# jkbonfield/htscodecs

Hardware: AMD Instinct MI355X
Metric: MB/s uncompressed throughput (encode+decode), rANS4x16 order-1, q40 blocks (higher is better)
Workload: dtype u8/u32; 1 GPU; rANS4x16 order-1 encode+decode, 23040 x 1048576 B q40+dir blocks per GPU (cyclic tiles of tests/dat/q40+dir), device-resident; order=1, blocks_per_gpu=23040, block_size=1048576

## Files before the change

### htscodecs_amd/csrc/r4x16_enc_chain.h

```cpp
#pragma once
#include <stdlib.h>
#include <type_traits>
#include "r4x16_dev.h"
#include "r4x16_sched.h"
#include "r4x16_enc_step.h"

template <int ORDER>
__device__ __forceinline__ u32 chain_encode(gcu8 *data, u32 n, gcu8 *image, u32 ns, u32 bits, gcu32 *rcptab,
                                            gu8 *scratch_end, bool active, u32 lane)
{
    const u32 k = lane & 3;
    GAS const u16 *cum = (GAS const u16 *)(image + ENC_IMG_IDX);
    const u32 rs = ns + 1;
    u32 x = RANS_LOW;
    u32 written = 0;
    u32 nsteps, first;
    u32 p;
    const u32 q = n >> 2;
    if (ORDER == 0) {
        const u32 gtop = n ? (n - 1) >> 2 : 0;
        nsteps = n ? gtop + 1 : 0;
        first = (4 * gtop + k < n) ? 0 : 1;
        p = 4 * (gtop - (first ? 1 : 0)) + k;
    } else {
        const u32 tail = n - 4 * q;
        nsteps = tail + q;
        first = (k == 3) ? 0 : tail;
        p = (k == 3) ? n - 1 : k * q + q - 1;
    }
    if (!active) { nsteps = 0; first = 0; }

    u32 cur = 0;
    if (nsteps > first) cur = image[data[p]];

    for (u32 s = 0; wave_any(s < nsteps); s++) {
        const bool live = s >= first && s < nsteps;
        bool emit = false;
        u32 rcp = 0, pk = 0, nextc = 0;
        if (live) {
            u32 row = 0;
            if (ORDER == 0) {
                if (p >= 4) nextc = image[data[p - 4]];
            } else if (s != nsteps - 1) {
                nextc = image[data[p - 1]];
                row = nextc;
            }
            const u32 c0 = cum[row * rs + cur], c1 = cum[row * rs + cur + 1];
            pk = c0 | ((c1 - c0) << 16);
            rcp = enc_rcp(rcptab, c1 - c0);
            emit = enc_wants_emit(x, pk, bits);
        }
        const u32 em = quad_ballot(emit, lane);
        if (emit) {
            const u32 above = __popc(em >> (k + 1));
            *(gu16 *)(scratch_end - 2 * (written + above + 1)) = (u16)x;
            x >>= 16;
        }
        written += __popc(em);
        if (live) {
            x = enc_advance(x, rcp, pk, bits);
            cur = nextc;
            p -= (ORDER == 0) ? 4 : 1;
        }
    }
    if (active) *(gu32 *)(scratch_end - 2 * written - 16 + 4 * k) = x;
    return active ? 2 * written + 16 : 0;
}

#define ENC_LRCP_BYTES 16400u
#define ENC_LFREQ_BYTES   8208u
static_assert(ENC_LFREQ_BYTES >= 8u * ENC_FREQTAB_ENTRIES && ENC_LFREQ_BYTES % 16u == 0, "frequency table in LDS");
template <bool BYTE>
struct EncOutT {
    u8 *ring;
    u32 ring126;
    gu8 *send;
    gu8 *dump;
    u32 written;
    u32 flushed;
    u32 k, lane;
    bool active;
    u32x4 held;
    gu8 *held_dst;
    u32 above = (0xeu << k) & 0xfu;
    static constexpr u32 HALF_SHIFT = BYTE ? 6u : 5u;
    __device__ __forceinline__ u32 emit16(u32 x, bool live, bool over)
    {
        const u64 m = __ballot(over) & __ballot(live);
        const u32 em = (u32)(m >> (lane & ~3u)) & 0xfu;
        const bool emit = live && over;
        const u32 j = written + __popc(em >> (k + 1));
        const u32 j63 = emit ? (j & 63u) : ~0u;
        *(LAS u16 *)(unsigned long)(ring126 - 2u * j63) = (u16)x;
        written += __popc(em);
        return emit ? x >> 16 : x;
    }
    template <bool ALL>
    __device__ __forceinline__ u32 emit16q(u32 x, bool live, bool over)
    {
        const u64 m = ALL ? __ballot(over) : __ballot(over) & __ballot(live);
        const u32 em = (u32)(m >> (lane & ~3u));
        const bool emit = ALL ? over : live && over;
        const u32 j = written + __popc(em & above);
        const u32 j63 = emit ? (j & 63u) : ~0u;
        u32 a;
        asm("v_mad_i32_i24 %0, %1, -2, %2" : "=v"(a) : "v"(j63), "v"(ring126));
        *(LAS u16 *)(unsigned long)a = (u16)x;
        written += __popc(em & 0xfu);
        return emit ? x >> 16 : x;
    }
    template <bool Q = false, bool ALL = false>
    __device__ __forceinline__ void step(u32 &x, bool live, u32 rcp, u32 pk, u32 bits)
    {
        const u32 f = pk >> 16, start = pk & 0xffffu;
        u32 xs;
        if (BYTE) {
            const u32 x_max = f << 19;
            const bool o1 = x >= x_max, o2 = (x >> 8) >= x_max;
            const u64 lv = __ballot(live);
            const u32 e1 = (u32)((__ballot(o1) & lv) >> (lane & ~3u)) & 0xfu, e2 = (u32)((__ballot(o2) & lv) >> (lane & ~3u)) & 0xfu;
            const bool emit1 = live && o1, emit2 = live && o2;
            const u32 j = written + __popc(e1 >> (k + 1)) + __popc(e2 >> (k + 1));
            const u32 j1 = emit1 ? (j & 127u) : ~0u, j2 = emit2 ? ((j + 1u) & 127u) : ~0u;
            *(LAS u8 *)(unsigned long)(ring126 - j1) = (u8)x;
            *(LAS u8 *)(unsigned long)(ring126 - j2) = (u8)(x >> 8);
            xs = emit2 ? x >> 16 : emit1 ? x >> 8 : x;
            written += __popc(e1) + __popc(e2);
        } else xs = Q ? emit16q<ALL>(x, live, x >= (f << (31u - bits))) : emit16(x, live, x >= (f << (31u - bits)));
        const u32 fm1 = f - 1u;
        const u32 rsh = 31u - (u32)__clz((int)(fm1 | 1u));
        const u32 q = (__umulhi(xs, rcp) >> rsh) + (fm1 == 0u ? 1u : 0u);
        const u32 cmpl = (1u << bits) - f;
        const u32 xn = __umul24(q, cmpl) + (xs + start);
        x = ALL || live ? xn : xs;
    }
    template <bool ALL = false>
    __device__ __forceinline__ void step_freq(u32 &x, bool live, u32 m, u32 w, u32 start, u32 f)
    {
        const u32 xs = emit16q<ALL>(x, live, x >= (f << 21));
        const u32 q = (__umulhi(xs, m) + xs) >> ((w >> 24) & 31u);
        const u32 xn = __umul24(q, w) + (xs + start);
        x = ALL || live ? xn : xs;
    }
    __device__ __forceinline__ void flush()
    {
        const bool due = active && (written >> HALF_SHIFT) != flushed;
        if (wave_any(due)) {
            if (due) {
                const u32x4 v = *(const u32x4 *)(ring + ((flushed & 1u) ? 0u : 64u) + 16u * k);
                *(GAS u32x4_unaligned *)(send - 64ull * (flushed + 1u) + 16u * k) = v;
                flushed++;
            }
        }
    }
    __device__ __forceinline__ void flush_pipelined()
    {
        *(GAS u32x4_unaligned *)held_dst = held;
        const bool due = active && (written >> HALF_SHIFT) != flushed;
        held = *(const u32x4 *)(ring + ((flushed & 1u) ? 0u : 64u) + 16u * k);
        held_dst = due ? send - 64ull * (flushed + 1u) + 16u * k : dump;
        flushed += due ? 1u : 0u;
    }
    __device__ __forceinline__ void flush_drain()
    {
        *(GAS u32x4_unaligned *)held_dst = held;
        held_dst = dump;
    }
    __device__ __forceinline__ u32 finish(u32 x)
    {
        flush();
        if (BYTE) { flush(); }
        const u32 first = (BYTE ? 64u : 32u) * flushed;
        const u32 rem = active ? written - first : 0u;
        for (u32 i = k; wave_any(i < rem); i += 4) {
            if (i < rem) {
                const u32 j = first + i;
                if (BYTE) send[-(long)(j + 1u)] = *(const u8 *)(ring + (127u - (j & 127u)));
                else *(gu16 *)(send - 2ull * (j + 1u)) = *(const u16 *)(ring + ((~j << 1) & 126u));
            }
        }
        if (active) {
            if (BYTE) { gu8 *d = send - written - 16 + 4 * k; d[0] = (u8)x; d[1] = (u8)(x >> 8); d[2] = (u8)(x >> 16); d[3] = (u8)(x >> 24); }
            else *(gu32 *)(send - 2ull * written - 16 + 4 * k) = x;
        }
        return active ? (BYTE ? written : 2 * written) + 16 : 0;
    }
};
typedef EncOutT<false> EncOut;

template <bool PK, bool BYTE = false, bool FT = false>
__device__ __forceinline__ u32 chain_encode_o1_lds(const u8 *img_lds, u8 *ring, const u32 *lrcp, gcu8 *data, u32 n, u32 ns,
                                                   u32 bits, gcu8 *safe, gu8 *scratch_end, gu8 *dump, bool active, u32 lane,
                                                   bool aff_wave = false, u32 aff = 0u)
{
    const u32 k = lane & 3;
    static_assert(!FT || (PK && !BYTE), "the frequency table serves the packed rows");
    if (PK) bits = 10u;
    const u8 *idx = img_lds;
    const u8 *cumb = img_lds + (FT ? ENC_IMG_IDX_SHORT : ENC_IMG_IDX);
    const u32 rs = PK ? 4u * enc_pk_row_dwords(ns) : ns + 1;
    const u32 cumb_lds = (u32)(unsigned long)(LAS const u8 *)cumb;
    const u32 wmul = PK ? 11u | (rs >> 2) << 16 : 1u, wadd = PK ? (cumb_lds >> 2) << 16 : 0u;
    auto word = [&](u32 j) -> u32 {
        if (!PK) return j;
        u32 w = __umul24(j, wmul) + wadd;
        asm("" : "+v"(w));
        return w;
    };
    auto pairw = [&](u32 wc, u32 ws) -> u32 {
        if (PK) {
            const u32 a = ((wc >> 16) + __builtin_amdgcn_ubfe(ws, 5, 5)) << 2;
            const u32x2 d = *(LAS const u32x2_a4 *)(unsigned long)a;
            return __builtin_amdgcn_alignbit(d.y, d.x, ws);
        }
        return *(LAS const u32 *)(cumb + 2u * (__umul24(wc, rs) + ws));
    };
    auto pair = [&](u32 ci, u32 si) -> u32 { return pairw(word(ci), word(si)); };
    const u32 neutral = 1024u << 11;
    const u32 rcp_last = RCPTAB_ENTRIES - 1u;
    struct PF { u32 pk, f; };
    auto rcpof = [&](PF s) -> u32x2 {
        if (FT) return ((const u32x2 *)lrcp)[s.f];
        const u32 f = s.pk >> 16;
        u32x2 r = {lrcp[PK ? f : f < rcp_last ? f : rcp_last], 0u};
        return r;
    };
    auto topk = [&](u32 p) -> PF {
        if (PK) {
            const u32 st = p & 2047u, f = __builtin_amdgcn_ubfe(p, 11, 11) - st;
            PF r = {FT ? st : st | (f << 16), f};
            return r;
        }
        u32 hi = p << 16; asm("" : "+v"(hi));
        PF r = {p - hi, 0u};
        return r;
    };
    struct Sym { u32 rcp, w; PF s; };
    auto fetch = [&](u32 ci, u32 si) -> Sym {
        const PF s = topk(pair(ci, si));
        const u32x2 e = rcpof(s);
        Sym r = {e.x, e.y, s};
        return r;
    };
    auto step = [&](EncOutT<BYTE> &o, u32 &x, bool live, u32 rcp, u32 w, u32 pk, u32 f) {
        if (FT) o.step_freq(x, live, rcp, w, pk, f);
        else o.template step<PK>(x, live, rcp, pk, bits);
    };
    auto step_all = [&](EncOutT<BYTE> &o, u32 &x, u32 rcp, u32 w, u32 pk, u32 f) {
        if (FT) o.template step_freq<true>(x, true, rcp, w, pk, f);
        else o.template step<true, true>(x, true, rcp, pk, bits);
    };
    EncOutT<BYTE> o{ring, (u32)(unsigned long)(LAS u8 *)ring + (BYTE ? 127u : 126u), scratch_end, dump, 0u, 0u, k, lane, active, {0, 0, 0, 0}, dump};
    u32 x = BYTE ? (1u << 23) : RANS_LOW;
    const u32 q = active ? n >> 2 : 0;
    const u32 tail = active ? n - 4 * q : 0;

    u32 cur = 0;
    if (active && k == 3 && tail) cur = idx[data[n - 1]];
    for (u32 s = 0; wave_any(s < tail); s++) {
        const bool live = k == 3 && s < tail;
        Sym e = {0, 0, {0, 0}};
        if (live) {
            const u32 ci = idx[data[n - 2 - s]];
            e = fetch(ci, cur);
            cur = ci;
        }
        step(o, x, live, e.rcp, e.w, e.s.pk, e.s.f);
    }

    gcu8 *qbase = data + (u64)k * q;
    const u32 r0 = q ? q - 1 : 0;
    const u32 main = r0;
    const u32 npair = main >> 3;
    const u32 ntrip = 2 * npair;
    cur = (active && q) ? idx[qbase[r0]] : 0u;
    auto pipelined = [&](auto affc) {
        constexpr bool AFF = decltype(affc)::value;
        gcu8 *lbase = npair ? qbase : safe;
        u32 loff = npair ? r0 : 0u;
        auto load8 = [&](u32 j) -> u32x2 {
            if (!PK) {
                gcu8 *p = j < npair ? qbase + (r0 - 8 * j) - 8 : safe;
                return *(GAS const u32x2_unaligned *)p;
            }
            loff = __builtin_elementwise_sub_sat(loff, 8u);
            return *(GAS const u32x2_unaligned *)(lbase + loff);
        };
        struct I4 { u32 c0, c1, c2, c3; };
        u32 amul = 0u, aadd = wadd;
        if (AFF && npair) { amul = wmul; aadd = wadd - __umul24(aff - 1u, wmul); }
        auto aword = [&](u32 b) -> u32 {
            u32 w = __umul24(b, amul) + aadd;
            asm("" : "+v"(w));
            return w;
        };
        auto idx4 = [&](u32 ww) -> I4 {
            if (AFF) {
                I4 r = {aword(ww >> 24), aword((ww >> 16) & 0xff), aword((ww >> 8) & 0xff), aword(ww & 0xff)};
                return r;
            }
            I4 r = {word(idx[ww >> 24]), word(idx[(ww >> 16) & 0xff]), word(idx[(ww >> 8) & 0xff]), word(idx[ww & 0xff])};
            return r;
        };
        auto cum4 = [&](const I4 &c, u32 sym) -> u32x4 {
            u32x4 r = {pairw(c.c0, sym), pairw(c.c1, c.c0), pairw(c.c2, c.c1), pairw(c.c3, c.c2)};
            return r;
        };
        auto real4 = [&](u32x4 p, bool live) -> u32x4 {
            if (!PK) return p;
            u32x4 r = {live ? p.x : neutral, live ? p.y : neutral, live ? p.z : neutral, live ? p.w : neutral};
            return r;
        };
        struct P4 { PF x, y, z, w; };
        auto topk4 = [&](u32x4 p) -> P4 {
            P4 r = {topk(p.x), topk(p.y), topk(p.z), topk(p.w)};
            return r;
        };
        struct R4 { u32x4 rcp, w; };
        auto rcp4 = [&](const P4 &p) -> R4 {
            const u32x2 a = rcpof(p.x), b = rcpof(p.y), c = rcpof(p.z), d = rcpof(p.w);
            R4 r = {{a.x, b.x, c.x, d.x}, {a.y, b.y, c.y, d.y}};
            return r;
        };
        u32 cur1, cur2;
        I4 I2;
        P4 P0;
        u32x4 Praw;
        R4 R0;
        u32x2 Q0, Q1, Q2, Q3;
        {
            Q0 = load8(0); Q1 = load8(1); Q2 = load8(2); Q3 = load8(3);
            const I4 i0 = idx4(Q0.y), i1 = idx4(Q0.x);
            I2 = idx4(Q1.y);
            P0 = topk4(real4(cum4(i0, word(cur)), 0 < ntrip));
            Praw = cum4(i1, i0.c3);
            cur1 = i0.c3; cur2 = i1.c3;
            R0 = rcp4(P0);
        }
        u32 t = 0;
        auto trip = [&](u32 wnext3) {
            const bool live = t < ntrip;
            const I4 In = idx4(wnext3);
            const u32x4 Pn = cum4(I2, cur2);
            const P4 P1 = topk4(real4(Praw, t + 1 < ntrip));
            const R4 Rn = rcp4(P1);
            __builtin_amdgcn_sched_barrier(0);
            if (PK) {
                step_all(o, x, R0.rcp.x, R0.w.x, P0.x.pk, P0.x.f);
                step_all(o, x, R0.rcp.y, R0.w.y, P0.y.pk, P0.y.f);
                step_all(o, x, R0.rcp.z, R0.w.z, P0.z.pk, P0.z.f);
                step_all(o, x, R0.rcp.w, R0.w.w, P0.w.pk, P0.w.f);
            } else {
                step(o, x, live, R0.rcp.x, R0.w.x, P0.x.pk, P0.x.f);
                step(o, x, live, R0.rcp.y, R0.w.y, P0.y.pk, P0.y.f);
                step(o, x, live, R0.rcp.z, R0.w.z, P0.z.pk, P0.z.f);
                step(o, x, live, R0.rcp.w, R0.w.w, P0.w.pk, P0.w.f);
                if (live) cur = cur1;
            }
            cur1 = cur2; cur2 = I2.c3;
            I2 = In; P0 = P1; Praw = Pn; R0 = Rn;
            t++;
            __builtin_amdgcn_sched_barrier(0);
        };
        for (u32 d = 0; wave_any(d < npair); d += 4) {
            Q0 = load8(d + 4); o.flush_pipelined(); trip(Q1.x); trip(Q2.y);
            Q1 = load8(d + 5); o.flush_pipelined(); trip(Q2.x); trip(Q3.y);
            Q2 = load8(d + 6); o.flush_pipelined(); trip(Q3.x); trip(Q0.y);
            Q3 = load8(d + 7); o.flush_pipelined(); trip(Q0.x); trip(Q1.y);
        }
        o.flush_drain();
        o.flush();
        if (PK) cur = (active && q) ? idx[qbase[r0 - 4 * ntrip]] : 0u;
    };
    if (wave_any(npair > 0)) {
        if constexpr (FT) {
            if (aff_wave) pipelined(std::true_type{});
            else pipelined(std::false_type{});
        } else pipelined(std::false_type{});
    }
    u32 r = r0 - 4 * ntrip, done = 4 * ntrip;
    for (; wave_any(done < main); ) {
        const bool live = done < main;
        Sym e = {0, 0, {0, 0}};
        if (live) {
            const u32 ci = idx[qbase[r - 1]];
            e = fetch(ci, cur);
            cur = ci; r--; done++;
        }
        step(o, x, live, e.rcp, e.w, e.s.pk, e.s.f);
        o.flush();
    }
    {
        const bool live = active && q > 0;
        Sym e = {0, 0, {0, 0}};
        if (live) e = fetch(0, cur);
        step(o, x, live, e.rcp, e.w, e.s.pk, e.s.f);
    }
    return o.finish(x);
}

template <bool BYTE = false>
__device__ __forceinline__ u32 chain_encode_o0_pipe(const u8 *img_lds, u8 *ring, const u32 *lrcp, gcu8 *data, u32 n,
                                                    u32 bits, gcu8 *safe, gu8 *scratch_end, gu8 *dump, bool active, u32 lane)
{
    const u32 k = lane & 3;
    const u8 *idx = img_lds;
    const u8 *cumb = img_lds + ENC_IMG_IDX;
    auto pair = [&](u32 si) -> u32 { return *(LAS const u32 *)(cumb + 2u * si); };
    auto rcpof = [&](u32 pk) -> u32 { const u32 f = pk >> 16; return lrcp[f < RCPTAB_ENTRIES - 1u ? f : RCPTAB_ENTRIES - 1u]; };
    auto topk = [&](u32 p) -> u32 { u32 hi = p << 16; asm("" : "+v"(hi)); return p - hi; };
    auto fetch = [&](u32 si) -> u32x2 {
        const u32 pk = topk(pair(si));
        u32x2 r = {rcpof(pk), pk};
        return r;
    };
    EncOutT<BYTE> o{ring, (u32)(unsigned long)(LAS u8 *)ring + (BYTE ? 127u : 126u), scratch_end, dump, 0u, 0u, k, lane, active, {0, 0, 0, 0}, dump};
    u32 x = BYTE ? (1u << 23) : RANS_LOW;
    const u32 Q = active ? n >> 2 : 0;
    const u32 rem = active ? n & 3u : 0;

    if (wave_any(rem != 0)) {
        const bool live = k < rem;
        u32 rcp = 0, pk = 0;
        if (live) { const u32x2 e = fetch(idx[data[4 * Q + k]]); rcp = e.x; pk = e.y; }
        o.step(x, live, rcp, pk, bits);
    }

    const u32 npair = Q >> 3;
    const u32 ntrip = 2 * npair;
    if (wave_any(npair > 0)) {
        struct DT { u32x4 a, b; };
        auto load_dt = [&](u32 j) -> DT {
            gcu8 *p = j < npair ? data + 4ull * (Q - 8 * j) - 32 : safe;
            DT r = {*(GAS const u32x4_unaligned *)(p + 16), *(GAS const u32x4_unaligned *)p};
            return r;
        };
        struct I4 { u32 c0, c1, c2, c3; };
        const u32 sh = 8 * k;
        auto idx4 = [&](u32x4 v) -> I4 {
            I4 r = {idx[(v.w >> sh) & 0xff], idx[(v.z >> sh) & 0xff], idx[(v.y >> sh) & 0xff], idx[(v.x >> sh) & 0xff]};
            return r;
        };
        auto cum4 = [&](const I4 &c) -> u32x4 {
            u32x4 r = {pair(c.c0), pair(c.c1), pair(c.c2), pair(c.c3)};
            return r;
        };
        auto topk4 = [&](u32x4 p) -> u32x4 {
            u32x4 r = {topk(p.x), topk(p.y), topk(p.z), topk(p.w)};
            return r;
        };
        auto rcp4 = [&](u32x4 p) -> u32x4 {
            u32x4 r = {rcpof(p.x), rcpof(p.y), rcpof(p.z), rcpof(p.w)};
            return r;
        };
        I4 I2;
        u32x4 P0, Praw, R0;
        DT Q0, Q1, Q2, Q3;
        {
            Q0 = load_dt(0); Q1 = load_dt(1); Q2 = load_dt(2); Q3 = load_dt(3);
            const I4 i0 = idx4(Q0.a), i1 = idx4(Q0.b);
            I2 = idx4(Q1.a);
            P0 = topk4(cum4(i0));
            Praw = cum4(i1);
            R0 = rcp4(P0);
        }
        u32 t = 0;
        auto trip = [&](u32x4 wnext3) {
            const bool live = t < ntrip;
            const I4 In = idx4(wnext3);
            const u32x4 Pn = cum4(I2);
            const u32x4 P1 = topk4(Praw);
            const u32x4 Rn = rcp4(P1);
            __builtin_amdgcn_sched_barrier(0);
            o.step(x, live, R0.x, P0.x, bits);
            o.step(x, live, R0.y, P0.y, bits);
            o.step(x, live, R0.z, P0.z, bits);
            o.step(x, live, R0.w, P0.w, bits);
            I2 = In; P0 = P1; Praw = Pn; R0 = Rn;
            t++;
            __builtin_amdgcn_sched_barrier(0);
        };
        for (u32 d = 0; wave_any(d < npair); d += 4) {
            Q0 = load_dt(d + 4); o.flush_pipelined(); trip(Q1.b); trip(Q2.a);
            Q1 = load_dt(d + 5); o.flush_pipelined(); trip(Q2.b); trip(Q3.a);
            Q2 = load_dt(d + 6); o.flush_pipelined(); trip(Q3.b); trip(Q0.a);
            Q3 = load_dt(d + 7); o.flush_pipelined(); trip(Q0.b); trip(Q1.a);
        }
        o.flush_drain();
        o.flush();
    }
    for (u32 g = Q - 4 * ntrip; wave_any(g > 0); ) {
        const bool live = g > 0;
        u32 rcp = 0, pk = 0;
        if (live) { g--; const u32x2 e = fetch(idx[data[4 * g + k]]); rcp = e.x; pk = e.y; }
        o.step(x, live, rcp, pk, bits);
        o.flush();
    }
    return o.finish(x);
}


#define ENC_LRCP_PK_BYTES 4112u
template <bool LDS_IMG, bool PK, bool FT = false>
__global__ __launch_bounds__(256) void k_enc_chain(EncItem *items, const u32 *rcptab_, u8 *dump_, const u32 *list, u32 *count,
                                                   int qpw, int spw, u32 lds_per_item, int dyn, int aff_on, u32 *aff_count)
{
    extern __shared__ __attribute__((aligned(16))) u8 lds[];
    const u32 tid = threadIdx.x;
    const u32 lane = tid & (WAVE - 1);
    const u32 wq = lane >> 2;
    const u32 quad = (tid >> 6) * (u32)spw + wq;
    const int nmine = (int)count[SCHED_COUNT];
    list += count[SCHED_START];
    SchedWalk walk(count, nmine, qpw, dyn != 0);
    for (;;) {
    const int wg = LDS_IMG ? walk.next_wg((volatile u32 *)lds + 1) : walk.next_wave();
    if (wg < 0) break;
    const int slot = wg * qpw + (int)quad;
    const bool mine = wq < (u32)spw && quad < (u32)qpw && slot < nmine;
    EncItem *I = &items[mine ? list[slot] : list[wg * qpw]];
    bool active = mine && I->active;
    const u32 img_bytes = active ? I->img_bytes : 0u;
    if (LDS_IMG) {
        volatile u32 *flag = (volatile u32 *)lds;
        if (tid == 0) *flag = 0;
        __syncthreads();
        if (active) *flag = 1;
        __syncthreads();
        const u32 any = *flag;
        __syncthreads();
        if (!any) continue;
    } else if (!wave_any(active)) continue;
    sched_setprio(sched_prio_of(active, active ? I->n : 0u));

    const u32 order = active ? I->order : 2u;
    gcu32 *rcptab = to_global(rcptab_);
    gcu8 *data = (gcu8 *)I->data;
    gu8 *send = (gu8 *)I->scratch_end;
    const u32 n = I->n, ns = I->ns, bits = active ? I->bits : 12u;
    u32 pay;
    if (LDS_IMG) {
        u32 *lrcp = (u32 *)lds;
        u8 *slots = lds + (FT ? ENC_LFREQ_BYTES : PK ? ENC_LRCP_PK_BYTES : ENC_LRCP_BYTES);
        if (FT) for (u32 j = tid; j < 2u * ENC_FREQTAB_ENTRIES; j += blockDim.x) lrcp[j] = rcptab[ENC_FREQTAB_OFF + j];
        else for (u32 j = tid; j < (PK ? 1025u : RCPTAB_ENTRIES); j += blockDim.x) lrcp[j] = rcptab[j];
        const u64 my_img = active ? I->image : 0ull;
        const u32 wq0 = (tid >> 6) * (u32)spw;
        for (u32 qd = 0; qd < WAVE / 4; qd++) {
            const u64 src = __shfl(my_img, (int)qd * 4);
            const u32 nb = __shfl(img_bytes, (int)qd * 4);
            if (!src) continue;
            gcu32x4 *s = (gcu32x4 *)src;
            u32x4 *dd = (u32x4 *)(slots + (u64)(wq0 + qd) * lds_per_item);
            for (u32 j = lane; j < ((nb + 15) >> 4); j += WAVE) dd[j] = s[j];
        }
        __syncthreads();
        const u32 slot = active ? quad : 0u;
        const u8 *im = slots + (u64)slot * lds_per_item;
        u8 *ring = slots + (u64)slot * lds_per_item + (lds_per_item - ENC_RING_BYTES);
        gu8 *dump = to_global(dump_) + 16u * ((blockIdx.x * blockDim.x + tid) & (ENC_DUMP_BYTES / 16u - 1u));
        if (FT) {
            const u32 aff = !aff_on ? 0u : active ? I->affine : 1u;
            const bool aff_wave = !wave_any(aff == 0u);
            pay = chain_encode_o1_lds<PK, false, FT>(im, ring, lrcp, data, n, ns, bits, (gcu8 *)rcptab, send, dump, order == 1, lane, aff_wave, aff);
            const u32 nstreams = (u32)__popcll(__ballot(active) & 0x1111111111111111ull);
            if (aff_count && aff_wave && lane == 0) atomicAdd(aff_count, nstreams);
        } else pay = chain_encode_o1_lds<PK, false, FT>(im, ring, lrcp, data, n, ns, bits, (gcu8 *)rcptab, send, dump, order == 1, lane);
        if (!PK) pay |= chain_encode_o0_pipe(im, ring, lrcp, data, n, bits, (gcu8 *)rcptab, send, dump, order == 0, lane);
    } else {
        gcu8 *im = (gcu8 *)I->image;
        pay = chain_encode<1>(data, n, im, ns, bits, rcptab, send, order == 1, lane);
        pay |= chain_encode<0>(data, n, im, ns, bits, rcptab, send, order == 0, lane);
    }
    if (active && (lane & 3) == 0) I->pay_len = pay;
    if (LDS_IMG) __syncthreads();
    }
    walk.leave();
}
```

Before: 177,500 MB/s.

## Hand-schedule order-1 frequency-table encode trip in inline assembly

Adds a hand-written inline-assembly trip_freq that performs the four rANS encode steps of a trip, including renormalisation byte emission via ballot/popcount and LDS ring writes, in one tightly scheduled block. The frequency-table path now precomputes the renormalisation threshold with a single 24-bit multiply on the packed cum/freq word and uses it directly as an LDS address for the reciprocal entry. It also masks the start field late inside the asm so the masking fills scheduling gaps. The aim is to cut instruction count and dependency stalls in the encoder's hot loop. The cost is fragile hard-coded registers (v30:v31) and a strong reliance on the packed layout assumptions.

```diff
diff --git a/htscodecs_amd/csrc/r4x16_enc_chain.h b/htscodecs_amd/csrc/r4x16_enc_chain.h
--- a/htscodecs_amd/csrc/r4x16_enc_chain.h
+++ b/htscodecs_amd/csrc/r4x16_enc_chain.h
@@ -135,12 +135,51 @@
         x = ALL || live ? xn : xs;
     }
     template <bool ALL = false>
-    __device__ __forceinline__ void step_freq(u32 &x, bool live, u32 m, u32 w, u32 start, u32 f)
-    {
-        const u32 xs = emit16q<ALL>(x, live, x >= (f << 21));
+    __device__ __forceinline__ void step_freq(u32 &x, bool live, u32 m, u32 w, u32 start, u32 X)
+    {
+        const u32 xs = emit16q<ALL>(x, live, x >= X);
         const u32 q = (__umulhi(xs, m) + xs) >> ((w >> 24) & 31u);
         const u32 xn = __umul24(q, w) + (xs + start);
         x = ALL || live ? xn : xs;
+    }
+#define ENC_TRIP_EM    "v[30:31]"
+#define ENC_TRIP_EM_LO "v30"
+#define ENC_TRIP_EM_CLOBBER "v30", "v31"
+#define ENC_TRIP_WRITE(xp) \
+        "v_mad_i32_i24 %[q], %[pj], -2, %[r126]\n\t" \
+        "ds_write_b16 %[q], %[" xp "]\n\t"
+#define ENC_TRIP_STEP(gap, xi, xo, n) \
+        "v_cmp_ge_u32_e32 vcc, %[" xi "], %[X" n "]\n\t" \
+        gap \
+        "v_lshrrev_b64 " ENC_TRIP_EM ", %[sh], vcc\n\t" \
+        "v_cndmask_b32_sdwa %[xs], %[" xi "], %[" xi "], vcc dst_sel:DWORD dst_unused:UNUSED_PAD src0_sel:DWORD src1_sel:WORD_1\n\t" \
+        "v_and_b32_e32 %[t], %[above], " ENC_TRIP_EM_LO "\n\t" \
+        "v_mul_hi_u32 %[q], %[xs], %[m" n "]\n\t" \
+        "v_and_b32_e32 " ENC_TRIP_EM_LO ", 15, " ENC_TRIP_EM_LO "\n\t" \
+        "v_bcnt_u32_b32 %[t], %[t], %[wr]\n\t" \
+        "v_add_u32_e32 %[q], %[xs], %[q]\n\t" \
+        "v_bcnt_u32_b32 %[wr], " ENC_TRIP_EM_LO ", %[wr]\n\t" \
+        "v_lshrrev_b32_sdwa %[q], %[w" n "], %[q] dst_sel:DWORD dst_unused:UNUSED_PAD src0_sel:BYTE_3 src1_sel:DWORD\n\t" \
+        "v_and_b32_e32 %[t], 63, %[t]\n\t" \
+        "v_mul_u32_u24_e32 %[q], %[q], %[w" n "]\n\t" \
+        "v_cndmask_b32_e32 %[pj], -1, %[t], vcc\n\t" \
+        "v_add3_u32 %[" xo "], %[xs], %[s" n "], %[q]\n\t"
+    __device__ __forceinline__ void trip_freq(u32 &x, u32x4 m, u32x4 w, u32 s0, u32 s1, u32 s2, u32 s3, u32 X0, u32 X1, u32 X2, u32 X3,
+                                              u32 &na, u32 &nb)
+    {
+        u32 xb, xs, t, q, pj;
+        const u32 sh = lane & ~3u;
+        asm volatile(ENC_TRIP_STEP("v_and_b32_e32 %[na], 0x7ff, %[na]\n\t"
+                                   "v_and_b32_e32 %[nb], 0x7ff, %[nb]\n\t", "xa", "xb", "0")
+                     ENC_TRIP_STEP(ENC_TRIP_WRITE("xa"), "xb", "xa", "1")
+                     ENC_TRIP_STEP(ENC_TRIP_WRITE("xb"), "xa", "xb", "2")
+                     ENC_TRIP_STEP(ENC_TRIP_WRITE("xa"), "xb", "xa", "3")
+                     ENC_TRIP_WRITE("xb")
+                     : [xa] "+v"(x), [wr] "+v"(written), [na] "+v"(na), [nb] "+v"(nb), [xb] "=&v"(xb), [xs] "=&v"(xs), [t] "=&v"(t), [q] "=&v"(q), [pj] "=&v"(pj)
+                     : [sh] "v"(sh), [above] "v"(above), [r126] "v"(ring126),
+                       [m0] "v"(m.x), [w0] "v"(w.x), [s0] "v"(s0), [X0] "v"(X0), [m1] "v"(m.y), [w1] "v"(w.y), [s1] "v"(s1), [X1] "v"(X1),
+                       [m2] "v"(m.z), [w2] "v"(w.z), [s2] "v"(s2), [X2] "v"(X2), [m3] "v"(m.w), [w3] "v"(w.w), [s3] "v"(s3), [X3] "v"(X3)
+                     : "vcc", "memory", ENC_TRIP_EM_CLOBBER);
     }
     __device__ __forceinline__ void flush()
     {
@@ -207,10 +246,13 @@
         asm("" : "+v"(w));
         return w;
     };
+    auto pairr = [&](u32 wc, u32 ws) -> u32x2 {
+        const u32 a = ((wc >> 16) + __builtin_amdgcn_ubfe(ws, 5, 5)) << 2;
+        return *(LAS const u32x2_a4 *)(unsigned long)a;
+    };
     auto pairw = [&](u32 wc, u32 ws) -> u32 {
         if (PK) {
-            const u32 a = ((wc >> 16) + __builtin_amdgcn_ubfe(ws, 5, 5)) << 2;
-            const u32x2 d = *(LAS const u32x2_a4 *)(unsigned long)a;
+            const u32x2 d = pairr(wc, ws);
             return __builtin_amdgcn_alignbit(d.y, d.x, ws);
         }
         return *(LAS const u32 *)(cumb + 2u * (__umul24(wc, rs) + ws));
@@ -220,15 +262,22 @@
     const u32 rcp_last = RCPTAB_ENTRIES - 1u;
     struct PF { u32 pk, f; };
     auto rcpof = [&](PF s) -> u32x2 {
-        if (FT) return ((const u32x2 *)lrcp)[s.f];
+        if (FT) return *(LAS const u32x2 *)(unsigned long)(s.f >> 18);
         const u32 f = s.pk >> 16;
         u32x2 r = {lrcp[PK ? f : f < rcp_last ? f : rcp_last], 0u};
         return r;
     };
-    auto topk = [&](u32 p) -> PF {
+    int xmul = 1024 - 2097152;
+    if (FT) asm("" : "+s"(xmul));
+    auto topk = [&](u32 p, bool late = false) -> PF {
+        if (FT) {
+            const u32 X = (u32)__mul24((int)p, xmul);
+            PF r = {late ? p : p & 2047u, X & 0xffe00000u};
+            return r;
+        }
         if (PK) {
             const u32 st = p & 2047u, f = __builtin_amdgcn_ubfe(p, 11, 11) - st;
-            PF r = {FT ? st : st | (f << 16), f};
+            PF r = {st | (f << 16), f};
             return r;
         }
         u32 hi = p << 16; asm("" : "+v"(hi));
@@ -303,6 +352,18 @@
             return r;
         };
         auto cum4 = [&](const I4 &c, u32 sym) -> u32x4 {
+            if (FT) {
+                const u32x2 d0 = pairr(c.c0, sym), d1 = pairr(c.c1, c.c0), d2 = pairr(c.c2, c.c1), d3 = pairr(c.c3, c.c2);
+                u32x4 r;
+                asm("v_alignbit_b32 %0, %4, %5, %6\n\t"
+                    "v_alignbit_b32 %1, %7, %8, %9\n\t"
+                    "v_alignbit_b32 %2, %10, %11, %12\n\t"
+                    "v_alignbit_b32 %3, %13, %14, %15"
+                    : "=&v"(r.x), "=&v"(r.y), "=&v"(r.z), "=v"(r.w)
+                    : "v"(d0.y), "v"(d0.x), "v"(sym), "v"(d1.y), "v"(d1.x), "v"(c.c0), "v"(d2.y), "v"(d2.x), "v"(c.c1),
+                      "v"(d3.y), "v"(d3.x), "v"(c.c2));
+                return r;
+            }
             u32x4 r = {pairw(c.c0, sym), pairw(c.c1, c.c0), pairw(c.c2, c.c1), pairw(c.c3, c.c2)};
             return r;
         };
@@ -312,8 +373,8 @@
             return r;
         };
         struct P4 { PF x, y, z, w; };
-        auto topk4 = [&](u32x4 p) -> P4 {
-            P4 r = {topk(p.x), topk(p.y), topk(p.z), topk(p.w)};
+        auto topk4 = [&](u32x4 p, bool late = false) -> P4 {
+            P4 r = {topk(p.x, late), topk(p.y, late), topk(p.z), topk(p.w)};
             return r;
         };
         struct R4 { u32x4 rcp, w; };
@@ -342,10 +403,12 @@
             const bool live = t < ntrip;
             const I4 In = idx4(wnext3);
             const u32x4 Pn = cum4(I2, cur2);
-            const P4 P1 = topk4(real4(Praw, t + 1 < ntrip));
+            P4 P1 = topk4(real4(Praw, t + 1 < ntrip), FT);
             const R4 Rn = rcp4(P1);
             __builtin_amdgcn_sched_barrier(0);
-            if (PK) {
+            if (FT) {
+                o.trip_freq(x, R0.rcp, R0.w, P0.x.pk, P0.y.pk, P0.z.pk, P0.w.pk, P0.x.f, P0.y.f, P0.z.f, P0.w.f, P1.x.pk, P1.y.pk);
+            } else if (PK) {
                 step_all(o, x, R0.rcp.x, R0.w.x, P0.x.pk, P0.x.f);
                 step_all(o, x, R0.rcp.y, R0.w.y, P0.y.pk, P0.y.f);
                 step_all(o, x, R0.rcp.z, R0.w.z, P0.z.pk, P0.z.f);
```

Measured after the change: 180,500 MB/s (median of 6 runs). +1.7%, better.
